# Zeng-Yan/centermask2

Measured on AMD Instinct MI355X. Metric: images/sec whole-node (V2-39-eSE 3x800x1280), higher is better.
Workload: dtype f32; 1 GPU; Full CenterMask2 V-39-eSE (VoVNetV2-FPN + FCOS + CenterROIHeads/SAG-Mask/MaskIoU + ROIAlignV2), bs=8 per GPU, 3x800x1280, end-to-end (BASELINE configs[3]); global_batch=8, per_gpu_batch=8, parallelism=dp1, launch=hip-graph, collective=none, weights=seeded random-init, reference state-dict keys

## Files before the change

centermask2_amd/csrc/detect.hip:

```cpp
#include "cmk_common.hpp"

namespace cmk {

constexpr int SEL_CHUNK = 4096;
constexpr int MAX_LEVELS = 8;

struct SelLevels {
    const float* logits[MAX_LEVELS];
    const float* regctr[MAX_LEVELS];
    int W[MAX_LEVELS];
    int stride[MAX_LEVELS];
    int elems[MAX_LEVELS];
    int blk_begin[MAX_LEVELS + 1];
    int num_levels;
};

__device__ inline float sigmoidf_(float x) { return 1.0f / (1.0f + expf(-x)); }

__device__ inline int find_level(const SelLevels& L, int b) {
    int l = 0;
#pragma unroll
    for (int i = 1; i < MAX_LEVELS; ++i)
        if (i < L.num_levels && b >= L.blk_begin[i]) l = i;
    return l;
}

__device__ inline bool is_candidate(const float* lg, const float* rc, int e, int ne, int C, float thr, int with_ctr, float& p) {
    if (e >= ne) { p = 0.f; return false; }
    p = sigmoidf_(lg[e]);
    if (!with_ctr) return p > thr;
    return p * sigmoidf_(rc[(long)(e / C) * 5 + 4]) > thr;
}

__global__ __launch_bounds__(256) void sel_count_kernel(const SelLevels L, int C, float thr, int with_ctr, int32_t* __restrict__ block_counts) {
    const int b = blockIdx.x, n = blockIdx.y;
    const int l = find_level(L, b);
    const int e0 = (b - L.blk_begin[l]) * SEL_CHUNK;
    const int ne = L.elems[l];
    const float* lg = L.logits[l] + (long)n * ne;
    const float* rc = L.regctr[l] + (long)n * (ne / C) * 5;
    const int lane = threadIdx.x & 63, wave = threadIdx.x >> 6;
    int cnt = 0;
#pragma unroll 4
    for (int it = 0; it < 16; ++it) {
        int e = e0 + wave * 1024 + it * 64 + lane;
        float p;
        bool c = is_candidate(lg, rc, e, ne, C, thr, with_ctr, p);
        cnt += __popcll(__ballot(c));
    }
    __shared__ int wc[4];
    if (lane == 0) wc[wave] = cnt;
    __syncthreads();
    if (threadIdx.x == 0) block_counts[(long)n * gridDim.x + b] = wc[0] + wc[1] + wc[2] + wc[3];
}

__global__ __launch_bounds__(256) void sel_scan_kernel(int32_t* __restrict__ block_counts, int blocks_per_image, int32_t* __restrict__ counts) {
    __shared__ int part[256];
    const int n = blockIdx.x;
    int32_t* bc = block_counts + (long)n * blocks_per_image;
    const int per = cdiv(blocks_per_image, 256);
    const int b0 = threadIdx.x * per, b1 = min(blocks_per_image, b0 + per);
    int s = 0;
    for (int b = b0; b < b1; ++b) s += bc[b];
    part[threadIdx.x] = s;
    __syncthreads();
    if (threadIdx.x == 0) {
        int run = 0;
        for (int i = 0; i < 256; ++i) { int v = part[i]; part[i] = run; run += v; }
        counts[n] = run;
    }
    __syncthreads();
    int run = part[threadIdx.x];
    for (int b = b0; b < b1; ++b) { int v = bc[b]; bc[b] = run; run += v; }
}

__global__ __launch_bounds__(256) void sel_write_kernel(const SelLevels L, int C, float thr, int with_ctr, const int32_t* __restrict__ block_offsets,
                                                       float* __restrict__ cand_box, float* __restrict__ cand_score,
                                                       int32_t* __restrict__ cand_cls, float* __restrict__ cand_loc, int cap) {
    const int b = blockIdx.x, n = blockIdx.y;
    const int l = find_level(L, b);
    const int e0 = (b - L.blk_begin[l]) * SEL_CHUNK;
    const int ne = L.elems[l];
    const float* lg = L.logits[l] + (long)n * ne;
    const float* rc = L.regctr[l] + (long)n * (ne / C) * 5;
    const int Wl = L.W[l];
    const float fstride = (float)L.stride[l];
    const float half = (float)(L.stride[l] / 2);
    const int lane = threadIdx.x & 63, wave = threadIdx.x >> 6;
    const unsigned long long lt = (lane == 0) ? 0ull : (~0ull >> (64 - lane));

    int cnt = 0;
    for (int it = 0; it < 16; ++it) {
        int e = e0 + wave * 1024 + it * 64 + lane;
        float p;
        bool c = is_candidate(lg, rc, e, ne, C, thr, with_ctr, p);
        cnt += __popcll(__ballot(c));
    }
    __shared__ int wc[4];
    if (lane == 0) wc[wave] = cnt;
    __syncthreads();
    int base = block_offsets[(long)n * gridDim.x + b];
    for (int w = 0; w < wave; ++w) base += wc[w];

    for (int it = 0; it < 16; ++it) {
        int e = e0 + wave * 1024 + it * 64 + lane;
        float p;
        const bool c = is_candidate(lg, rc, e, ne, C, thr, with_ctr, p);
        unsigned long long m = __ballot(c);
        int dst = base + __popcll(m & lt);
        base += __popcll(m);
        if (c && dst < cap) {
            int loc = e / C, cls = e - loc * C;
            const float* r = rc + (long)loc * 5;
            float ctr = sigmoidf_(r[4]);
            float score = sqrtf(p * ctr);
            float lx = (float)((loc % Wl) * L.stride[l]) + half;
            float ly = (float)((loc / Wl) * L.stride[l]) + half;
            float r0 = r[0] * fstride, r1 = r[1] * fstride, r2 = r[2] * fstride, r3 = r[3] * fstride;
            long o = (long)n * cap + dst;
            cand_box[o * 4 + 0] = lx - r0;
            cand_box[o * 4 + 1] = ly - r1;
            cand_box[o * 4 + 2] = lx + r2;
            cand_box[o * 4 + 3] = ly + r3;
            cand_score[o] = score;
            cand_cls[o] = cls;
            cand_loc[o * 2 + 0] = lx;
            cand_loc[o * 2 + 1] = ly;
        }
    }
}

constexpr int NT = 1024;
constexpr int NW = NT / 64;
constexpr int MAXK = 1024;

__device__ inline float iou_f(float ax1, float ay1, float ax2, float ay2, float aarea, float bx1, float by1, float bx2, float by2,
                              float barea) {
    float xx1 = fmaxf(ax1, bx1), yy1 = fmaxf(ay1, by1);
    float xx2 = fminf(ax2, bx2), yy2 = fminf(ay2, by2);
    float w = fmaxf(0.0f, xx2 - xx1), h = fmaxf(0.0f, yy2 - yy1);
    float inter = w * h;
    return inter / (aarea + barea - inter);
}

__global__ __launch_bounds__(NT) void nms_topk_kernel(const float* __restrict__ cand_box, const float* __restrict__ cand_score,
                                                     const int32_t* __restrict__ cand_cls, const float* __restrict__ cand_loc,
                                                     const int32_t* __restrict__ counts, int cap, float thr, int topk,
                                                     float* __restrict__ out_box, float* __restrict__ out_score,
                                                     int64_t* __restrict__ out_cls, float* __restrict__ out_loc,
                                                     int32_t* __restrict__ out_idx, int32_t* __restrict__ out_count,
                                                     uint32_t* __restrict__ sort_ws) {
    __shared__ int hist[256];
    __shared__ int base[256];
    __shared__ int wcnt[NW][256];
    __shared__ float red[NW];
    __shared__ float s_maxc;
    __shared__ float kx1[MAXK], ky1[MAXK], kx2[MAXK], ky2[MAXK], karea[MAXK];
    __shared__ int kcls[MAXK];
    __shared__ int s_nkept;

    const int n = blockIdx.x;
    const int tid = threadIdx.x, lane = tid & 63, wave = tid >> 6;
    const int cnt = min(counts[n], cap);
    const float* box = cand_box + (long)n * cap * 4;
    const float* score = cand_score + (long)n * cap;
    const int32_t* cls = cand_cls + (long)n * cap;
    uint32_t* k0 = sort_ws + ((long)n * 4 + 0) * cap;
    uint32_t* v0 = sort_ws + ((long)n * 4 + 1) * cap;
    uint32_t* k1 = sort_ws + ((long)n * 4 + 2) * cap;
    uint32_t* v1 = sort_ws + ((long)n * 4 + 3) * cap;

    float lmax = -INFINITY;
    for (int i = tid; i < cnt; i += NT) {
        k0[i] = ~__float_as_uint(score[i]);
        v0[i] = (uint32_t)i;
        const float* b = box + (long)i * 4;
        lmax = fmaxf(lmax, fmaxf(fmaxf(b[0], b[1]), fmaxf(b[2], b[3])));
    }
    lmax = wave_max(lmax);
    if (lane == 0) red[wave] = lmax;
    __syncthreads();
    if (tid == 0) {
        float m = red[0];
        for (int w = 1; w < NW; ++w) m = fmaxf(m, red[w]);
        s_maxc = m;
        s_nkept = 0;
    }
    __syncthreads();

    const unsigned long long lt = (lane == 0) ? 0ull : (~0ull >> (64 - lane));
    const int NEED = max(2048, 16 * topk);
    int sorted_cnt = cnt;
    for (int attempt = (cnt > 2 * NEED ? 0 : 1); attempt < 2; ++attempt) {
    uint32_t *kin = k0, *vin = v0, *kout = k1, *vout = v1;
    sorted_cnt = cnt;
    if (attempt == 1 && cnt > 2 * NEED) {
        for (int i = tid; i < cnt; i += NT) { k0[i] = ~__float_as_uint(score[i]); v0[i] = (uint32_t)i; }
        __threadfence_block();
        __syncthreads();
    }
    if (attempt == 0) {
        int* hist12 = &wcnt[0][0];
        for (int j = tid; j < 4096; j += NT) hist12[j] = 0;
        __syncthreads();
        for (int i = tid; i < cnt; i += NT) atomicAdd(&hist12[k0[i] >> 20], 1);
        __syncthreads();
        const int h0 = hist12[4 * tid], h1 = hist12[4 * tid + 1], h2 = hist12[4 * tid + 2], h3 = hist12[4 * tid + 3];
        const int mine = h0 + h1 + h2 + h3;
        int incl = mine;
#pragma unroll
        for (int o = 1; o < 64; o <<= 1) { int v = __shfl_up(incl, o, 64); if (lane >= o) incl += v; }
        if (lane == 63) base[wave] = incl;
        __syncthreads();
        int pre = incl - mine;
        for (int w = 0; w < wave; ++w) pre += base[w];
        if (pre < NEED && pre + mine >= NEED) {
            int c = pre + h0, d = 4 * tid;
            if (c < NEED) { c += h1; ++d; }
            if (c < NEED) { c += h2; ++d; }
            if (c < NEED) { c += h3; ++d; }
            hist[0] = d;
            hist[1] = c;
        }
        __syncthreads();
        const uint32_t dmax = (uint32_t)hist[0];
        sorted_cnt = hist[1];
        __syncthreads();
        int run = 0;
        for (int t0 = 0; t0 < cnt; t0 += NT) {
            const int i = t0 + tid;
            const bool take = i < cnt && (k0[i] >> 20) <= dmax;
            const unsigned long long bm = __ballot(take);
            if (lane == 0) base[wave] = __popcll(bm);
            __syncthreads();
            int pos = run + __popcll(bm & lt);
            for (int w = 0; w < wave; ++w) pos += base[w];
            if (take) { k1[pos] = k0[i]; v1[pos] = (uint32_t)i; }
            int tot = 0;
            for (int w = 0; w < NW; ++w) tot += base[w];
            run += tot;
            __syncthreads();
        }
        __threadfence_block();
        __syncthreads();
        kin = k1; vin = v1; kout = k0; vout = v0;
    }
    const int scnt = sorted_cnt;
    for (int pass = 0; pass < 4; ++pass) {
        const int shift = pass * 8;
        if (tid < 256) hist[tid] = 0;
        __syncthreads();
        for (int i = tid; i < scnt; i += NT) atomicAdd(&hist[(kin[i] >> shift) & 255], 1);
        __syncthreads();
        if (tid == 0) {
            int run = 0;
            for (int d = 0; d < 256; ++d) { base[d] = run; run += hist[d]; }
        }
        __syncthreads();
        const bool trivial = false;
        (void)trivial;
        for (int t0 = 0; t0 < scnt; t0 += NT) {
            for (int j = tid; j < NW * 256; j += NT) (&wcnt[0][0])[j] = 0;
            __syncthreads();
            const int i = t0 + tid;
            const bool valid = i < scnt;
            uint32_t key = valid ? kin[i] : 0u, val = valid ? vin[i] : 0u;
            int digit = valid ? (int)((key >> shift) & 255) : 256;
            unsigned long long peers = __ballot(valid);
#pragma unroll
            for (int bit = 0; bit < 8; ++bit) {
                unsigned long long bm = __ballot((digit >> bit) & 1);
                peers &= ((digit >> bit) & 1) ? bm : ~bm;
            }
            int rank = __popcll(peers & lt);
            if (valid && rank == 0) wcnt[wave][digit] = __popcll(peers);
            __syncthreads();
            if (valid) {
                int pre = base[digit];
                for (int w = 0; w < wave; ++w) pre += wcnt[w][digit];
                kout[pre + rank] = key;
                vout[pre + rank] = val;
            }
            __syncthreads();
            if (tid < 256) {
                int s = 0;
                for (int w = 0; w < NW; ++w) s += wcnt[w][tid];
                base[tid] += s;
            }
            __syncthreads();
        }
        uint32_t* t;
        t = kin; kin = kout; kout = t;
        t = vin; vin = vout; vout = t;
        __threadfence_block();
        __syncthreads();
    }
    const uint32_t* order = vin;

    if (wave == 0) {
        const bool per_class = cnt >= 40000;
        const float off_unit = per_class ? 0.0f : (s_maxc + 1.0f);
        int nkept = 0;
        for (int c0 = 0; c0 < scnt && nkept < topk; c0 += 64) {
            const int pos = c0 + lane;
            bool alive = pos < scnt;
            int idx = alive ? (int)order[pos] : 0;
            float x1 = 0, y1 = 0, x2 = 0, y2 = 0, area = 0;
            int mycls = -1;
            if (alive) {
                const float* b = box + (long)idx * 4;
                mycls = cls[idx];
                float off = (float)mycls * off_unit;
                x1 = b[0] + off; y1 = b[1] + off; x2 = b[2] + off; y2 = b[3] + off;
                area = (x2 - x1) * (y2 - y1);
                for (int k = 0; k < nkept; ++k) {
                    if (per_class && kcls[k] != mycls) continue;
                    if (iou_f(kx1[k], ky1[k], kx2[k], ky2[k], karea[k], x1, y1, x2, y2, area) > thr) { alive = false; break; }
                }
            }
            for (int t = 0; t < 64 && nkept < topk; ++t) {
                unsigned long long am = __ballot(alive);
                if (!((am >> t) & 1ull)) continue;
                float tx1 = __shfl(x1, t, 64), ty1 = __shfl(y1, t, 64), tx2 = __shfl(x2, t, 64), ty2 = __shfl(y2, t, 64);
                float tarea = __shfl(area, t, 64);
                int tcls = __shfl(mycls, t, 64);
                int tidx = __shfl(idx, t, 64);
                if (lane == 0) {
                    kx1[nkept] = tx1; ky1[nkept] = ty1; kx2[nkept] = tx2; ky2[nkept] = ty2; karea[nkept] = tarea; kcls[nkept] = tcls;
                    long o = (long)n * topk + nkept;
                    const float* b = box + (long)tidx * 4;
                    out_box[o * 4 + 0] = b[0]; out_box[o * 4 + 1] = b[1]; out_box[o * 4 + 2] = b[2]; out_box[o * 4 + 3] = b[3];
                    out_score[o] = score[tidx];
                    out_cls[o] = (int64_t)tcls;
                    out_loc[o * 2 + 0] = cand_loc[((long)n * cap + tidx) * 2 + 0];
                    out_loc[o * 2 + 1] = cand_loc[((long)n * cap + tidx) * 2 + 1];
                    out_idx[o] = tidx;
                }
                ++nkept;
                if (lane > t && alive && (!per_class || tcls == mycls) &&
                    iou_f(tx1, ty1, tx2, ty2, tarea, x1, y1, x2, y2, area) > thr)
                    alive = false;
                if (lane == t) alive = false;
            }
        }
        if (lane == 0) {
            out_count[n] = nkept;
            s_nkept = nkept;
        }
    }
    __syncthreads();
    if (s_nkept >= topk || sorted_cnt >= cnt) break;
    __syncthreads();
    }
    __syncthreads();
    for (int k = s_nkept + tid; k < topk; k += NT) {
        long o = (long)n * topk + k;
        out_box[o * 4 + 0] = out_box[o * 4 + 1] = out_box[o * 4 + 2] = out_box[o * 4 + 3] = 0.f;
        out_score[o] = 0.f;
        out_cls[o] = 0;
        out_loc[o * 2] = out_loc[o * 2 + 1] = 0.f;
        out_idx[o] = -1;
    }
}

static int fill_levels(const cmk_fcos_level* levels, int num_levels, int C, SelLevels& L) {
    if (num_levels < 1 || num_levels > MAX_LEVELS) return -1;
    int blk = 0;
    L.num_levels = num_levels;
    for (int l = 0; l < MAX_LEVELS; ++l) {
        if (l < num_levels) {
            long e = (long)levels[l].H * levels[l].W * C;
            if (e <= 0 || e > 0x7fffffffL) return -1;
            L.logits[l] = levels[l].logits; L.regctr[l] = levels[l].regctr;
            L.W[l] = levels[l].W; L.stride[l] = levels[l].stride; L.elems[l] = (int)e;
            L.blk_begin[l] = blk;
            blk += (int)((e + SEL_CHUNK - 1) / SEL_CHUNK);
        } else {
            L.logits[l] = nullptr; L.regctr[l] = nullptr; L.W[l] = 1; L.stride[l] = 1; L.elems[l] = 0; L.blk_begin[l] = blk;
        }
    }
    L.blk_begin[MAX_LEVELS] = blk;
    return blk;
}

}

using namespace cmk;

extern "C" int64_t cmk_fcos_select_ws_len(const cmk_fcos_level* levels, int num_levels, int N, int C) {
    SelLevels L;
    int blk = fill_levels(levels, num_levels, C, L);
    return blk < 0 ? -1 : (int64_t)blk * N;
}

extern "C" int cmk_fcos_select(const cmk_fcos_level* levels, int num_levels, int N, int C, float pre_nms_thresh, int thresh_with_ctr, float* cand_box,
                               float* cand_score, int32_t* cand_cls, float* cand_loc, int32_t* counts, int32_t* block_counts,
                               int64_t block_counts_len, int cap, void* stream) {
    if (!levels || !cand_box || !cand_score || !cand_cls || !cand_loc || !counts || !block_counts)
        return fail(CMK_EINVAL, "fcos_select: null pointer%s", "");
    if (N < 1 || C < 1 || cap < 1) return fail(CMK_EINVAL, "fcos_select: bad sizes%s", "");
    SelLevels L;
    int blk = fill_levels(levels, num_levels, C, L);
    if (blk < 0) return fail(CMK_EINVAL, "fcos_select: bad level table%s", "");
    for (int l = 0; l < num_levels; ++l)
        if (!levels[l].logits || !levels[l].regctr) return fail(CMK_EINVAL, "fcos_select: null level pointer%s", "");
    if (block_counts_len < (int64_t)blk * N) return fail(CMK_EINVAL, "fcos_select: workspace too small%s", "");
    hipStream_t st = (hipStream_t)stream;
    hipLaunchKernelGGL(sel_count_kernel, dim3(blk, N), dim3(256), 0, st, L, C, pre_nms_thresh, thresh_with_ctr, block_counts);
    int rc = check_launch("sel_count");
    if (rc) return rc;
    hipLaunchKernelGGL(sel_scan_kernel, dim3(N), dim3(256), 0, st, block_counts, blk, counts);
    rc = check_launch("sel_scan");
    if (rc) return rc;
    hipLaunchKernelGGL(sel_write_kernel, dim3(blk, N), dim3(256), 0, st, L, C, pre_nms_thresh, thresh_with_ctr, block_counts, cand_box, cand_score,
                       cand_cls, cand_loc, cap);
    return check_launch("sel_write");
}

extern "C" int cmk_nms_topk(const float* cand_box, const float* cand_score, const int32_t* cand_cls, const float* cand_loc,
                            const int32_t* counts, int N, int cap, float iou_thr, int topk, float* out_box, float* out_score,
                            int64_t* out_cls, float* out_loc, int32_t* out_idx, int32_t* out_count, uint32_t* sort_ws, void* stream) {
    if (!cand_box || !cand_score || !cand_cls || !cand_loc || !counts || !out_box || !out_score || !out_cls || !out_loc || !out_idx ||
        !out_count || !sort_ws)
        return fail(CMK_EINVAL, "nms_topk: null pointer%s", "");
    if (N < 1 || cap < 1 || topk < 1 || topk > MAXK) return fail(CMK_EINVAL, "nms_topk: need 1 <= topk <= %s%ld", "", (long)MAXK);
    hipLaunchKernelGGL(nms_topk_kernel, dim3(N), dim3(NT), 0, (hipStream_t)stream, cand_box, cand_score, cand_cls, cand_loc, counts, cap,
                       iou_thr, topk, out_box, out_score, out_cls, out_loc, out_idx, out_count, sort_ws);
    return check_launch("nms_topk");
}
```

centermask2_amd/csrc/elementwise.hip:

```cpp
#include "cmk_common.hpp"

namespace cmk {

typedef float f32x4 __attribute__((ext_vector_type(4)));
typedef float f32x16 __attribute__((ext_vector_type(16)));

template <int NB>
__global__ __launch_bounds__(256) void stem_conv_kernel(const float* __restrict__ x, const float* __restrict__ w,
                                                       const float* __restrict__ scale, const float* __restrict__ shift,
                                                       float* __restrict__ y, int N, int H, int W, int Ho, int Wo, long tiles) {
    const int lane = threadIdx.x & 63, wave = threadIdx.x >> 6;
    const int li = lane & 31, hh = lane >> 5;
    constexpr int Cout = NB * 32;
    float b[14][NB], sc[NB], sh[NB];
    int dlt[14], khs[14], kws[14];
#pragma unroll
    for (int s = 0; s < 14; ++s) {
        const int k = 2 * s + hh;
        const int ci = k % 3, t = k / 3, kw = t % 3, kh = t / 3;
        khs[s] = kh - 1; kws[s] = kw - 1;
        dlt[s] = (ci * H + kh - 1) * W + kw - 1;
#pragma unroll
        for (int nb = 0; nb < NB; ++nb) b[s][nb] = k < 27 ? w[k * Cout + nb * 32 + li] : 0.f;
    }
#pragma unroll
    for (int nb = 0; nb < NB; ++nb) { sc[nb] = scale[nb * 32 + li]; sh[nb] = shift[nb * 32 + li]; }
    const long total = (long)N * Ho * Wo;
    const long hw = (long)Ho * Wo;
    for (long tile = (long)blockIdx.x * 4 + wave; tile < tiles; tile += (long)gridDim.x * 4) {
        const long pix = tile * 32 + li;
        const bool pv = pix < total;
        const int n = (int)(pix / hw);
        const int rem = (int)(pix - (long)n * hw);
        const int oh = rem / Wo, ow = rem - oh * Wo;
        const int ih0 = oh * 2, iw0 = ow * 2;
        const float* xb = x + ((long)n * 3 * H + ih0) * W + iw0;
        float av[14];
#pragma unroll
        for (int s = 0; s < 14; ++s) {
            const int ih = ih0 + khs[s], iw = iw0 + kws[s];
            const bool ok = pv && (2 * s + hh < 27) && ih >= 0 && ih < H && iw >= 0 && iw < W;
            av[s] = ok ? xb[dlt[s]] : 0.f;
        }
        f32x16 acc[NB];
#pragma unroll
        for (int nb = 0; nb < NB; ++nb)
#pragma unroll
            for (int r = 0; r < 16; ++r) acc[nb][r] = 0.f;
#pragma unroll
        for (int s = 0; s < 14; ++s)
#pragma unroll
            for (int nb = 0; nb < NB; ++nb) acc[nb] = __builtin_amdgcn_mfma_f32_32x32x2f32(av[s], b[s][nb], acc[nb], 0, 0, 0);
#pragma unroll
        for (int r = 0; r < 16; ++r) {
            const long op = tile * 32 + (r & 3) + 8 * (r >> 2) + 4 * hh;
            if (op < total) {
#pragma unroll
                for (int nb = 0; nb < NB; ++nb) y[op * Cout + nb * 32 + li] = fmaxf(acc[nb][r] * sc[nb] + sh[nb], 0.f);
            }
        }
    }
}

__global__ __launch_bounds__(256) void maxpool3_kernel(const float* __restrict__ x, int x_cs, int x_co, float* __restrict__ y,
                                                      int y_cs, int y_co, int N, int H, int W, int Ho, int Wo, int C4,
                                                      const float* __restrict__ gate) {
    long total = (long)N * Ho * Wo * C4;
    for (long i = (long)blockIdx.x * 256 + threadIdx.x; i < total; i += (long)gridDim.x * 256) {
        int c4 = (int)(i % C4);
        long p = i / C4;
        int ow = (int)(p % Wo);
        int oh = (int)((p / Wo) % Ho);
        int n = (int)(p / ((long)Wo * Ho));
        f32x4 m = {-INFINITY, -INFINITY, -INFINITY, -INFINITY};
#pragma unroll
        for (int kh = 0; kh < 3; ++kh)
#pragma unroll
            for (int kw = 0; kw < 3; ++kw) {
                int ih = oh * 2 + kh, iw = ow * 2 + kw;
                if (ih < H && iw < W) {
                    f32x4 v = *reinterpret_cast<const f32x4*>(x + (((long)n * H + ih) * W + iw) * x_cs + x_co + c4 * 4);
                    m.x = fmaxf(m.x, v.x); m.y = fmaxf(m.y, v.y); m.z = fmaxf(m.z, v.z); m.w = fmaxf(m.w, v.w);
                }
            }
        if (gate) {
            f32x4 g = *reinterpret_cast<const f32x4*>(gate + ((long)n * C4 + c4) * 4);
            m.x *= g.x; m.y *= g.y; m.z *= g.z; m.w *= g.w;
        }
        *reinterpret_cast<f32x4*>(y + p * y_cs + y_co + c4 * 4) = m;
    }
}

__global__ __launch_bounds__(256) void subsample2_kernel(const float* __restrict__ x, int x_cs, int x_co, float* __restrict__ y, int y_cs, int y_co,
                                                        int N, int H, int W, int Ho, int Wo, int C4) {
    long total = (long)N * Ho * Wo * C4;
    for (long i = (long)blockIdx.x * 256 + threadIdx.x; i < total; i += (long)gridDim.x * 256) {
        int c4 = (int)(i % C4);
        long p = i / C4;
        int ow = (int)(p % Wo);
        int oh = (int)((p / Wo) % Ho);
        int n = (int)(p / ((long)Wo * Ho));
        *reinterpret_cast<f32x4*>(y + p * y_cs + y_co + c4 * 4) =
            *reinterpret_cast<const f32x4*>(x + (((long)n * H + 2 * oh) * W + 2 * ow) * x_cs + x_co + c4 * 4);
    }
}

__global__ __launch_bounds__(256) void ese_partial_kernel(const float* __restrict__ x, int x_cs, int x_co, float* __restrict__ ws,
                                                         int HW, int C, int chunks) {
    extern __shared__ float red[];
    const int n = blockIdx.y, chunk = blockIdx.x;
    const int G = C >> 2;
    const int ppl = G >= 256 ? 1 : 256 / G;
    const int per = cdiv(HW, chunks);
    const int p0 = chunk * per, p1 = min(HW, p0 + per);
    const float* xn = x + (long)n * HW * x_cs + x_co;
    for (int gi = threadIdx.x; gi < G * ppl; gi += 256) {
        int g = gi % G, pl = gi / G;
        f32x4 s = {0.f, 0.f, 0.f, 0.f};
        for (int p = p0 + pl; p < p1; p += ppl) {
            f32x4 v = *reinterpret_cast<const f32x4*>(xn + (long)p * x_cs + g * 4);
            s.x += v.x; s.y += v.y; s.z += v.z; s.w += v.w;
        }
        *reinterpret_cast<f32x4*>(red + pl * C + g * 4) = s;
    }
    __syncthreads();
    for (int c = threadIdx.x; c < C; c += 256) {
        float s = 0.f;
        for (int pl = 0; pl < ppl; ++pl) s += red[pl * C + c];
        ws[((long)n * chunks + chunk) * C + c] = s;
    }
}

__global__ __launch_bounds__(256) void ese_fc_kernel(const float* __restrict__ ws, const float* __restrict__ fc_w,
                                                    const float* __restrict__ fc_b, float* __restrict__ gate, int HW, int C,
                                                    int chunks) {
    extern __shared__ double smd[];
    const int n = blockIdx.y;
    const int G = C >> 2;
    const int parts = G >= 256 ? 1 : 256 / G;
    const float* wsn = ws + (long)n * chunks * C;
    for (int gi = threadIdx.x; gi < G * parts; gi += 256) {
        const int g = gi % G, part = gi / G;
        double s0 = 0.0, s1 = 0.0, s2 = 0.0, s3 = 0.0;
#pragma unroll 8
        for (int k = part; k < chunks; k += parts) {
            const f32x4 v = *reinterpret_cast<const f32x4*>(wsn + (long)k * C + g * 4);
            s0 += (double)v.x; s1 += (double)v.y; s2 += (double)v.z; s3 += (double)v.w;
        }
        double* o = smd + part * C + g * 4;
        o[0] = s0; o[1] = s1; o[2] = s2; o[3] = s3;
    }
    __syncthreads();
    for (int c = threadIdx.x; c < C; c += 256) {
        double s = 0.0;
        for (int part = 0; part < parts; ++part) s += smd[part * C + c];
        smd[c] = s / (double)HW;
    }
    __syncthreads();
    const int lane = threadIdx.x & 63, wave = threadIdx.x >> 6;
    for (int o = blockIdx.x * 16 + wave; o < min(C, (int)(blockIdx.x + 1) * 16); o += 4) {
        const float* wr = fc_w + (long)o * C;
        double s = 0.0;
        for (int c = lane * 4; c < C; c += 256) {
            f32x4 wv = *reinterpret_cast<const f32x4*>(wr + c);
            s += (double)wv.x * smd[c] + (double)wv.y * smd[c + 1] + (double)wv.z * smd[c + 2] + (double)wv.w * smd[c + 3];
        }
        s = wave_sum(s);
        if (lane == 0) {
            float v = (float)(s + (double)fc_b[o] + 3.0);
            gate[(long)n * C + o] = fminf(fmaxf(v, 0.f), 6.f) / 6.0f;
        }
    }
}

__global__ __launch_bounds__(256) void ese_fc_pooled_kernel(const float* __restrict__ rec, int rows, const float* __restrict__ fc_w,
                                                           const float* __restrict__ fc_b, float* __restrict__ gate, int HW, int C) {
    extern __shared__ double smd[];
    const int n = blockIdx.y;
    const int G = C >> 2;
    const int parts = G >= 256 ? 1 : 256 / G;
    const long p0 = (long)n * HW;
    const long g0 = p0 / rows, g1 = (p0 + HW - 1) / rows;
    const long first = (g0 * rows == p0) ? 2 * g0 : 2 * g0 + 1;
    for (int gi = threadIdx.x; gi < G * parts; gi += 256) {
        const int g = gi % G, part = gi / G;
        double s0 = 0.0, s1 = 0.0, s2 = 0.0, s3 = 0.0;
        if (part == 0) {
            const f32x4 v = *reinterpret_cast<const f32x4*>(rec + first * C + g * 4);
            s0 = v.x; s1 = v.y; s2 = v.z; s3 = v.w;
        }
#pragma unroll 8
        for (long k = g0 + 1 + part; k <= g1; k += parts) {
            const f32x4 v = *reinterpret_cast<const f32x4*>(rec + 2 * k * C + g * 4);
            s0 += (double)v.x; s1 += (double)v.y; s2 += (double)v.z; s3 += (double)v.w;
        }
        double* o = smd + part * C + g * 4;
        o[0] = s0; o[1] = s1; o[2] = s2; o[3] = s3;
    }
    __syncthreads();
    for (int c = threadIdx.x; c < C; c += 256) {
        double s = 0.0;
        for (int part = 0; part < parts; ++part) s += smd[part * C + c];
        smd[c] = s / (double)HW;
    }
    __syncthreads();
    const int lane = threadIdx.x & 63, wave = threadIdx.x >> 6;
    for (int o = blockIdx.x * 16 + wave; o < min(C, (int)(blockIdx.x + 1) * 16); o += 4) {
        const float* wr = fc_w + (long)o * C;
        double s = 0.0;
        for (int c = lane * 4; c < C; c += 256) {
            f32x4 wv = *reinterpret_cast<const f32x4*>(wr + c);
            s += (double)wv.x * smd[c] + (double)wv.y * smd[c + 1] + (double)wv.z * smd[c + 2] + (double)wv.w * smd[c + 3];
        }
        s = wave_sum(s);
        if (lane == 0) {
            float v = (float)(s + (double)fc_b[o] + 3.0);
            gate[(long)n * C + o] = fminf(fmaxf(v, 0.f), 6.f) / 6.0f;
        }
    }
}

__global__ __launch_bounds__(256) void ese_scale_kernel(const float* __restrict__ x, int x_cs, int x_co, const float* __restrict__ gate,
                                                       const float* __restrict__ idn, int id_cs, int id_co, float* __restrict__ y,
                                                       int y_cs, int y_co, int N, int HW, int C4) {
    long total = (long)N * HW * C4;
    for (long i = (long)blockIdx.x * 256 + threadIdx.x; i < total; i += (long)gridDim.x * 256) {
        int c4 = (int)(i % C4);
        long p = i / C4;
        int n = (int)(p / HW);
        f32x4 v = *reinterpret_cast<const f32x4*>(x + p * x_cs + x_co + c4 * 4);
        f32x4 g = *reinterpret_cast<const f32x4*>(gate + (long)n * C4 * 4 + c4 * 4);
        f32x4 o = {v.x * g.x, v.y * g.y, v.z * g.z, v.w * g.w};
        if (idn) {
            f32x4 d = *reinterpret_cast<const f32x4*>(idn + p * id_cs + id_co + c4 * 4);
            o.x += d.x; o.y += d.y; o.z += d.z; o.w += d.w;
        }
        *reinterpret_cast<f32x4*>(y + p * y_cs + y_co + c4 * 4) = o;
    }
}

}

using namespace cmk;

extern "C" int cmk_stem_conv_nchw3(const float* x, const float* w, const float* scale, const float* shift, float* y, int N, int H,
                                   int W, int Cout, void* stream) {
    if (!x || !w || !scale || !shift || !y) return fail(CMK_EINVAL, "stem: null pointer%s", "");
    if (Cout != 32 && Cout != 64 && Cout != 128) return fail(CMK_EINVAL, "stem: Cout (%s%ld) must be 32, 64 or 128", "", (long)Cout);
    int Ho = (H - 1) / 2 + 1, Wo = (W - 1) / 2 + 1;
    long total = (long)N * Ho * Wo;
    if ((long)3 * H * W >= (1L << 31)) return fail(CMK_EINVAL, "stem: image too large%s", "");
    long tiles = (total + 31) / 32;
    unsigned grid = (unsigned)std::min<long>((tiles + 3) / 4, 256 * 16);
    if (Cout == 32)
        hipLaunchKernelGGL(stem_conv_kernel<1>, dim3(grid), dim3(256), 0, (hipStream_t)stream, x, w, scale, shift, y, N, H, W, Ho, Wo, tiles);
    else if (Cout == 64)
        hipLaunchKernelGGL(stem_conv_kernel<2>, dim3(grid), dim3(256), 0, (hipStream_t)stream, x, w, scale, shift, y, N, H, W, Ho, Wo, tiles);
    else
        hipLaunchKernelGGL(stem_conv_kernel<4>, dim3(grid), dim3(256), 0, (hipStream_t)stream, x, w, scale, shift, y, N, H, W, Ho, Wo, tiles);
    return check_launch("stem_conv");
}

extern "C" int cmk_maxpool3x3s2_ceil_nhwc(const float* x, int x_cs, int x_co, float* y, int y_cs, int y_co, int N, int H, int W, int C,
                                          const float* gate, void* stream) {
    if (!x || !y) return fail(CMK_EINVAL, "maxpool: null pointer%s", "");
    if ((C & 3) || (x_cs & 3) || (x_co & 3) || (y_cs & 3) || (y_co & 3)) return fail(CMK_EINVAL, "maxpool: channels must be multiples of 4%s", "");
    if (H < 3 || W < 3) return fail(CMK_EINVAL, "maxpool: input smaller than the window%s", "");
    int Ho = (H - 3 + 1) / 2 + 1, Wo = (W - 3 + 1) / 2 + 1;
    if ((Ho - 1) * 2 >= H) --Ho;
    if ((Wo - 1) * 2 >= W) --Wo;
    long total = (long)N * Ho * Wo * (C >> 2);
    hipLaunchKernelGGL(maxpool3_kernel, dim3(stream_grid(total)), dim3(256), 0, (hipStream_t)stream, x, x_cs, x_co, y, y_cs, y_co, N, H, W,
                       Ho, Wo, C >> 2, gate);
    return check_launch("maxpool3");
}

extern "C" int cmk_maxpool1x1s2_nhwc(const float* x, int x_cs, int x_co, float* y, int y_cs, int y_co, int N, int H, int W, int C, void* stream) {
    if (!x || !y) return fail(CMK_EINVAL, "maxpool1x1s2: null pointer%s", "");
    if ((C & 3) || (x_cs & 3) || (x_co & 3) || (y_cs & 3) || (y_co & 3) || N < 1 || H < 1 || W < 1)
        return fail(CMK_EINVAL, "maxpool1x1s2: channels must be multiples of 4, N, H, W >= 1%s", "");
    const int Ho = (H - 1) / 2 + 1, Wo = (W - 1) / 2 + 1;
    long total = (long)N * Ho * Wo * (C >> 2);
    hipLaunchKernelGGL(subsample2_kernel, dim3(stream_grid(total)), dim3(256), 0, (hipStream_t)stream, x, x_cs, x_co, y, y_cs, y_co, N, H, W, Ho, Wo,
                       C >> 2);
    return check_launch("maxpool1x1s2");
}

extern "C" int cmk_ese_gate(const float* x, int x_cs, int x_co, const float* fc_w, const float* fc_b, float* gate, float* ws,
                            int ws_chunks, int N, int HW, int C, void* stream) {
    if (!x || !fc_w || !fc_b || !gate || !ws) return fail(CMK_EINVAL, "ese_gate: null pointer%s", "");
    if ((C & 3) || (x_cs & 3) || (x_co & 3) || ws_chunks < 1) return fail(CMK_EINVAL, "ese_gate: bad shape%s", "");
    int G = C >> 2;
    int ppl = G >= 256 ? 1 : 256 / G;
    size_t lds1 = (size_t)ppl * C * sizeof(float);
    hipLaunchKernelGGL(ese_partial_kernel, dim3(ws_chunks, N), dim3(256), lds1, (hipStream_t)stream, x, x_cs, x_co, ws, HW, C, ws_chunks);
    int rc = check_launch("ese_partial");
    if (rc) return rc;
    hipLaunchKernelGGL(ese_fc_kernel, dim3(cdiv(C, 16), N), dim3(256), 2 * lds1 , (hipStream_t)stream, ws, fc_w, fc_b,
                       gate, HW, C, ws_chunks);
    return check_launch("ese_fc");
}

extern "C" int cmk_ese_gate_pooled(const float* pool_ws, int rows, const float* fc_w, const float* fc_b, float* gate, int N, int HW, int C, void* stream) {
    if (!pool_ws || !fc_w || !fc_b || !gate) return fail(CMK_EINVAL, "ese_gate_pooled: null pointer%s", "");
    if ((C & 3) || rows < 1 || HW < rows || N < 1) return fail(CMK_EINVAL, "ese_gate_pooled: bad shape (C %% 4, H*W >= rows)%s", "");
    const int G = C >> 2;
    const int parts = G >= 256 ? 1 : 256 / G;
    hipLaunchKernelGGL(ese_fc_pooled_kernel, dim3(cdiv(C, 16), N), dim3(256), (size_t)parts * C * sizeof(double), (hipStream_t)stream, pool_ws, rows,
                       fc_w, fc_b, gate, HW, C);
    return check_launch("ese_fc_pooled");
}

extern "C" int cmk_ese_scale(const float* x, int x_cs, int x_co, const float* gate, const float* identity, int id_cs, int id_co, float* y,
                             int y_cs, int y_co, int N, int HW, int C, void* stream) {
    if (!x || !gate || !y) return fail(CMK_EINVAL, "ese_scale: null pointer%s", "");
    if ((C & 3) || (x_cs & 3) || (x_co & 3) || (y_cs & 3) || (y_co & 3) || (id_cs & 3) || (id_co & 3))
        return fail(CMK_EINVAL, "ese_scale: channels must be multiples of 4%s", "");
    long total = (long)N * HW * (C >> 2);
    hipLaunchKernelGGL(ese_scale_kernel, dim3(stream_grid(total)), dim3(256), 0, (hipStream_t)stream, x, x_cs, x_co, gate, identity, id_cs,
                       id_co, y, y_cs, y_co, N, HW, C >> 2);
    return check_launch("ese_scale");
}

__global__ __launch_bounds__(256) void upsample2x_add_kernel(float* __restrict__ y, const float* __restrict__ c, int N, int H, int W, int Hc, int Wc, int C4) {
    long total = (long)N * H * W * C4;
    for (long i = (long)blockIdx.x * 256 + threadIdx.x; i < total; i += (long)gridDim.x * 256) {
        int c4 = (int)(i % C4);
        long p = i / C4;
        int w = (int)(p % W);
        int h = (int)((p / W) % H);
        int n = (int)(p / ((long)W * H));
        const f32x4 a = *reinterpret_cast<const f32x4*>(y + i * 4);
        const f32x4 b = *reinterpret_cast<const f32x4*>(c + ((((long)n * Hc + (h >> 1)) * Wc + (w >> 1)) * C4 + c4) * 4);
        *reinterpret_cast<f32x4*>(y + i * 4) = f32x4{a.x + b.x, a.y + b.y, a.z + b.z, a.w + b.w};
    }
}

extern "C" int cmk_upsample2x_add_nhwc(float* y, const float* coarse, int N, int H, int W, int Hc, int Wc, int C, void* stream) {
    if (!y || !coarse) return fail(CMK_EINVAL, "upsample2x_add: null pointer%s", "");
    if ((C & 3) || N < 1 || H < 1 || W < 1 || Hc * 2 < H || Wc * 2 < W) return fail(CMK_EINVAL, "upsample2x_add: C %% 4 == 0 and a coarse map of at least half the size%s", "");
    long total = (long)N * H * W * (C >> 2);
    hipLaunchKernelGGL(upsample2x_add_kernel, dim3(stream_grid(total)), dim3(256), 0, (hipStream_t)stream, y, coarse, N, H, W, Hc, Wc, C >> 2);
    return check_launch("upsample2x_add");
}
```

Baseline: 374.1 images/sec.

## Fuse radix histograms into the load pass and cut barriers in NMS and eSE FC

The NMS top-k kernel now builds all four 8-bit radix histograms in the same pass that loads keys or compacts them, and scans them once instead of re-counting per pass. The prefix compaction uses a two-pass per-wave count and write with no per-chunk barriers, and reads scores directly rather than staging keys first. Kept-box output writes are deferred to a parallel loop after NMS, and the wave-serial candidate loop now jumps to set bits with ffs. Separately, the eSE FC gate computation processes four outputs per wave with unrolled weight loads, and the pooled reduction batches 16 loads per iteration to expose more memory parallelism. These kernels are a small part of the end-to-end detector, so their effect on whole-model throughput is limited.

```diff
diff --git a/centermask2_amd/csrc/detect.hip b/centermask2_amd/csrc/detect.hip
--- a/centermask2_amd/csrc/detect.hip
+++ b/centermask2_amd/csrc/detect.hip
@@ -150,13 +150,14 @@
                                                      int64_t* __restrict__ out_cls, float* __restrict__ out_loc,
                                                      int32_t* __restrict__ out_idx, int32_t* __restrict__ out_count,
                                                      uint32_t* __restrict__ sort_ws) {
-    __shared__ int hist[256];
-    __shared__ int base[256];
+    __shared__ int hist4[4][256];
+    __shared__ int sel[2];
+    __shared__ int wtot[NW];
     __shared__ int wcnt[NW][256];
     __shared__ float red[NW];
     __shared__ float s_maxc;
     __shared__ float kx1[MAXK], ky1[MAXK], kx2[MAXK], ky2[MAXK], karea[MAXK];
-    __shared__ int kcls[MAXK];
+    __shared__ int kcls[MAXK], kidx[MAXK];
     __shared__ int s_nkept;
 
     const int n = blockIdx.x;
@@ -169,16 +170,31 @@
     uint32_t* v0 = sort_ws + ((long)n * 4 + 1) * cap;
     uint32_t* k1 = sort_ws + ((long)n * 4 + 2) * cap;
     uint32_t* v1 = sort_ws + ((long)n * 4 + 3) * cap;
-
+    int* hist12 = &wcnt[0][0];
+
+    const int NEED = max(2048, 16 * topk);
+    const bool try_prefix = cnt > 2 * NEED;
+
+    for (int j = tid; j < NW * 256; j += NT) hist12[j] = 0;
+    (&hist4[0][0])[tid] = 0;
+    __syncthreads();
     float lmax = -INFINITY;
     for (int i = tid; i < cnt; i += NT) {
-        k0[i] = ~__float_as_uint(score[i]);
-        v0[i] = (uint32_t)i;
+        const uint32_t key = ~__float_as_uint(score[i]);
+        if (try_prefix) {
+            atomicAdd(&hist12[key >> 20], 1);
+        } else {
+            k0[i] = key;
+            v0[i] = (uint32_t)i;
+            atomicAdd(&hist4[0][key & 255], 1); atomicAdd(&hist4[1][(key >> 8) & 255], 1);
+            atomicAdd(&hist4[2][(key >> 16) & 255], 1); atomicAdd(&hist4[3][key >> 24], 1);
+        }
         const float* b = box + (long)i * 4;
         lmax = fmaxf(lmax, fmaxf(fmaxf(b[0], b[1]), fmaxf(b[2], b[3])));
     }
     lmax = wave_max(lmax);
     if (lane == 0) red[wave] = lmax;
+    __threadfence_block();
     __syncthreads();
     if (tid == 0) {
         float m = red[0];
@@ -189,79 +205,91 @@
     __syncthreads();
 
     const unsigned long long lt = (lane == 0) ? 0ull : (~0ull >> (64 - lane));
-    const int NEED = max(2048, 16 * topk);
     int sorted_cnt = cnt;
-    for (int attempt = (cnt > 2 * NEED ? 0 : 1); attempt < 2; ++attempt) {
+    for (int attempt = (try_prefix ? 0 : 1); attempt < 2; ++attempt) {
     uint32_t *kin = k0, *vin = v0, *kout = k1, *vout = v1;
     sorted_cnt = cnt;
-    if (attempt == 1 && cnt > 2 * NEED) {
-        for (int i = tid; i < cnt; i += NT) { k0[i] = ~__float_as_uint(score[i]); v0[i] = (uint32_t)i; }
+    if (attempt == 1 && try_prefix) {
+        (&hist4[0][0])[tid] = 0;
+        __syncthreads();
+        for (int i = tid; i < cnt; i += NT) {
+            const uint32_t key = ~__float_as_uint(score[i]);
+            k0[i] = key;
+            v0[i] = (uint32_t)i;
+            atomicAdd(&hist4[0][key & 255], 1); atomicAdd(&hist4[1][(key >> 8) & 255], 1);
+            atomicAdd(&hist4[2][(key >> 16) & 255], 1); atomicAdd(&hist4[3][key >> 24], 1);
+        }
         __threadfence_block();
         __syncthreads();
     }
     if (attempt == 0) {
-        int* hist12 = &wcnt[0][0];
-        for (int j = tid; j < 4096; j += NT) hist12[j] = 0;
-        __syncthreads();
-        for (int i = tid; i < cnt; i += NT) atomicAdd(&hist12[k0[i] >> 20], 1);
-        __syncthreads();
         const int h0 = hist12[4 * tid], h1 = hist12[4 * tid + 1], h2 = hist12[4 * tid + 2], h3 = hist12[4 * tid + 3];
         const int mine = h0 + h1 + h2 + h3;
         int incl = mine;
 #pragma unroll
         for (int o = 1; o < 64; o <<= 1) { int v = __shfl_up(incl, o, 64); if (lane >= o) incl += v; }
-        if (lane == 63) base[wave] = incl;
+        if (lane == 63) wtot[wave] = incl;
         __syncthreads();
         int pre = incl - mine;
-        for (int w = 0; w < wave; ++w) pre += base[w];
+        for (int w = 0; w < wave; ++w) pre += wtot[w];
         if (pre < NEED && pre + mine >= NEED) {
             int c = pre + h0, d = 4 * tid;
             if (c < NEED) { c += h1; ++d; }
             if (c < NEED) { c += h2; ++d; }
             if (c < NEED) { c += h3; ++d; }
-            hist[0] = d;
-            hist[1] = c;
-        }
-        __syncthreads();
-        const uint32_t dmax = (uint32_t)hist[0];
-        sorted_cnt = hist[1];
-        __syncthreads();
-        int run = 0;
-        for (int t0 = 0; t0 < cnt; t0 += NT) {
-            const int i = t0 + tid;
-            const bool take = i < cnt && (k0[i] >> 20) <= dmax;
+            sel[0] = d;
+            sel[1] = c;
+        }
+        hist12[4 * tid] = 0; hist12[4 * tid + 1] = 0; hist12[4 * tid + 2] = 0; hist12[4 * tid + 3] = 0;
+        __syncthreads();
+        const uint32_t dmax = (uint32_t)sel[0];
+        sorted_cnt = sel[1];
+        const int per = ((cnt + NW * 64 - 1) / (NW * 64)) * 64;
+        const int wb = min(cnt, wave * per), we = min(cnt, wb + per);
+        int mycount = 0;
+        for (int i0 = wb; i0 < we; i0 += 64) {
+            const int i = i0 + lane;
+            const bool take = i < we && ((~__float_as_uint(score[min(i, we - 1)])) >> 20) <= dmax;
+            mycount += __popcll(__ballot(take));
+        }
+        if (lane == 0) wtot[wave] = mycount;
+        __syncthreads();
+        int pos = 0;
+        for (int w = 0; w < wave; ++w) pos += wtot[w];
+        for (int i0 = wb; i0 < we; i0 += 64) {
+            const int i = i0 + lane;
+            const uint32_t key = ~__float_as_uint(score[min(i, we - 1)]);
+            const bool take = i < we && (key >> 20) <= dmax;
             const unsigned long long bm = __ballot(take);
-            if (lane == 0) base[wave] = __popcll(bm);
-            __syncthreads();
-            int pos = run + __popcll(bm & lt);
-            for (int w = 0; w < wave; ++w) pos += base[w];
-            if (take) { k1[pos] = k0[i]; v1[pos] = (uint32_t)i; }
-            int tot = 0;
-            for (int w = 0; w < NW; ++w) tot += base[w];
-            run += tot;
-            __syncthreads();
+            if (take) {
+                const int p = pos + __popcll(bm & lt);
+                k1[p] = key;
+                v1[p] = (uint32_t)i;
+                atomicAdd(&hist4[0][key & 255], 1); atomicAdd(&hist4[1][(key >> 8) & 255], 1);
+                atomicAdd(&hist4[2][(key >> 16) & 255], 1); atomicAdd(&hist4[3][key >> 24], 1);
+            }
+            pos += __popcll(bm);
         }
         __threadfence_block();
         __syncthreads();
         kin = k1; vin = v1; kout = k0; vout = v0;
     }
     const int scnt = sorted_cnt;
+    if (wave < 4) {
+        int* h = hist4[wave];
+        const int a0 = h[4 * lane], a1 = h[4 * lane + 1], a2 = h[4 * lane + 2], a3 = h[4 * lane + 3];
+        const int mine = a0 + a1 + a2 + a3;
+        int incl = mine;
+#pragma unroll
+        for (int o = 1; o < 64; o <<= 1) { int v = __shfl_up(incl, o, 64); if (lane >= o) incl += v; }
+        const int pre = incl - mine;
+        h[4 * lane] = pre; h[4 * lane + 1] = pre + a0; h[4 * lane + 2] = pre + a0 + a1; h[4 * lane + 3] = pre + a0 + a1 + a2;
+    }
+    __syncthreads();
     for (int pass = 0; pass < 4; ++pass) {
         const int shift = pass * 8;
-        if (tid < 256) hist[tid] = 0;
-        __syncthreads();
-        for (int i = tid; i < scnt; i += NT) atomicAdd(&hist[(kin[i] >> shift) & 255], 1);
-        __syncthreads();
-        if (tid == 0) {
-            int run = 0;
-            for (int d = 0; d < 256; ++d) { base[d] = run; run += hist[d]; }
-        }
-        __syncthreads();
-        const bool trivial = false;
-        (void)trivial;
+        int* base = hist4[pass];
         for (int t0 = 0; t0 < scnt; t0 += NT) {
-            for (int j = tid; j < NW * 256; j += NT) (&wcnt[0][0])[j] = 0;
-            __syncthreads();
             const int i = t0 + tid;
             const bool valid = i < scnt;
             uint32_t key = valid ? kin[i] : 0u, val = valid ? vin[i] : 0u;
@@ -284,7 +312,7 @@
             __syncthreads();
             if (tid < 256) {
                 int s = 0;
-                for (int w = 0; w < NW; ++w) s += wcnt[w][tid];
+                for (int w = 0; w < NW; ++w) { s += wcnt[w][tid]; wcnt[w][tid] = 0; }
                 base[tid] += s;
             }
             __syncthreads();
@@ -318,23 +346,15 @@
                     if (iou_f(kx1[k], ky1[k], kx2[k], ky2[k], karea[k], x1, y1, x2, y2, area) > thr) { alive = false; break; }
                 }
             }
-            for (int t = 0; t < 64 && nkept < topk; ++t) {
-                unsigned long long am = __ballot(alive);
-                if (!((am >> t) & 1ull)) continue;
+            for (unsigned long long am = __ballot(alive); am != 0ull && nkept < topk; am = __ballot(alive)) {
+                const int t = __ffsll((long long)am) - 1;
                 float tx1 = __shfl(x1, t, 64), ty1 = __shfl(y1, t, 64), tx2 = __shfl(x2, t, 64), ty2 = __shfl(y2, t, 64);
                 float tarea = __shfl(area, t, 64);
                 int tcls = __shfl(mycls, t, 64);
                 int tidx = __shfl(idx, t, 64);
                 if (lane == 0) {
                     kx1[nkept] = tx1; ky1[nkept] = ty1; kx2[nkept] = tx2; ky2[nkept] = ty2; karea[nkept] = tarea; kcls[nkept] = tcls;
-                    long o = (long)n * topk + nkept;
-                    const float* b = box + (long)tidx * 4;
-                    out_box[o * 4 + 0] = b[0]; out_box[o * 4 + 1] = b[1]; out_box[o * 4 + 2] = b[2]; out_box[o * 4 + 3] = b[3];
-                    out_score[o] = score[tidx];
-                    out_cls[o] = (int64_t)tcls;
-                    out_loc[o * 2 + 0] = cand_loc[((long)n * cap + tidx) * 2 + 0];
-                    out_loc[o * 2 + 1] = cand_loc[((long)n * cap + tidx) * 2 + 1];
-                    out_idx[o] = tidx;
+                    kidx[nkept] = tidx;
                 }
                 ++nkept;
                 if (lane > t && alive && (!per_class || tcls == mycls) &&
@@ -353,6 +373,17 @@
     __syncthreads();
     }
     __syncthreads();
+    for (int k = tid; k < s_nkept; k += NT) {
+        const long o = (long)n * topk + k;
+        const int tidx = kidx[k];
+        const float* b = box + (long)tidx * 4;
+        out_box[o * 4 + 0] = b[0]; out_box[o * 4 + 1] = b[1]; out_box[o * 4 + 2] = b[2]; out_box[o * 4 + 3] = b[3];
+        out_score[o] = score[tidx];
+        out_cls[o] = (int64_t)kcls[k];
+        out_loc[o * 2 + 0] = cand_loc[((long)n * cap + tidx) * 2 + 0];
+        out_loc[o * 2 + 1] = cand_loc[((long)n * cap + tidx) * 2 + 1];
+        out_idx[o] = tidx;
+    }
     for (int k = s_nkept + tid; k < topk; k += NT) {
         long o = (long)n * topk + k;
         out_box[o * 4 + 0] = out_box[o * 4 + 1] = out_box[o * 4 + 2] = out_box[o * 4 + 3] = 0.f;
diff --git a/centermask2_amd/csrc/elementwise.hip b/centermask2_amd/csrc/elementwise.hip
--- a/centermask2_amd/csrc/elementwise.hip
+++ b/centermask2_amd/csrc/elementwise.hip
@@ -131,6 +131,41 @@
     }
 }
 
+__device__ inline void ese_fc_outputs(const double* smd, const float* __restrict__ fc_w, const float* __restrict__ fc_b,
+                                      float* __restrict__ gate_n, int C) {
+    constexpr int NO = 4, KU = 4;
+    const int lane = threadIdx.x & 63, wave = threadIdx.x >> 6;
+    const int ob = blockIdx.x * 16 + wave;
+    double s[NO] = {0.0, 0.0, 0.0, 0.0};
+    for (int c0 = lane * 4; c0 < C; c0 += 256 * KU) {
+        f32x4 wv[NO][KU];
+#pragma unroll
+        for (int j = 0; j < NO; ++j)
+#pragma unroll
+            for (int k = 0; k < KU; ++k)
+                wv[j][k] = *reinterpret_cast<const f32x4*>(fc_w + (long)min(ob + 4 * j, C - 1) * C + min(c0 + 256 * k, C - 4));
+#pragma unroll
+        for (int k = 0; k < KU; ++k) {
+            const int c = c0 + 256 * k;
+            if (c < C) {
+#pragma unroll
+                for (int j = 0; j < NO; ++j)
+                    s[j] += (double)wv[j][k].x * smd[c] + (double)wv[j][k].y * smd[c + 1] + (double)wv[j][k].z * smd[c + 2] +
+                            (double)wv[j][k].w * smd[c + 3];
+            }
+        }
+    }
+#pragma unroll
+    for (int j = 0; j < NO; ++j) {
+        const int o = ob + 4 * j;
+        const double t = wave_sum(s[j]);
+        if (lane == 0 && o < min(C, (int)(blockIdx.x + 1) * 16)) {
+            float v = (float)(t + (double)fc_b[o] + 3.0);
+            gate_n[o] = fminf(fmaxf(v, 0.f), 6.f) / 6.0f;
+        }
+    }
+}
+
 __global__ __launch_bounds__(256) void ese_fc_kernel(const float* __restrict__ ws, const float* __restrict__ fc_w,
                                                     const float* __restrict__ fc_b, float* __restrict__ gate, int HW, int C,
                                                     int chunks) {
@@ -157,20 +192,7 @@
         smd[c] = s / (double)HW;
     }
     __syncthreads();
-    const int lane = threadIdx.x & 63, wave = threadIdx.x >> 6;
-    for (int o = blockIdx.x * 16 + wave; o < min(C, (int)(blockIdx.x + 1) * 16); o += 4) {
-        const float* wr = fc_w + (long)o * C;
-        double s = 0.0;
-        for (int c = lane * 4; c < C; c += 256) {
-            f32x4 wv = *reinterpret_cast<const f32x4*>(wr + c);
-            s += (double)wv.x * smd[c] + (double)wv.y * smd[c + 1] + (double)wv.z * smd[c + 2] + (double)wv.w * smd[c + 3];
-        }
-        s = wave_sum(s);
-        if (lane == 0) {
-            float v = (float)(s + (double)fc_b[o] + 3.0);
-            gate[(long)n * C + o] = fminf(fmaxf(v, 0.f), 6.f) / 6.0f;
-        }
-    }
+    ese_fc_outputs(smd, fc_w, fc_b, gate + (long)n * C, C);
 }
 
 __global__ __launch_bounds__(256) void ese_fc_pooled_kernel(const float* __restrict__ rec, int rows, const float* __restrict__ fc_w,
@@ -189,10 +211,13 @@
             const f32x4 v = *reinterpret_cast<const f32x4*>(rec + first * C + g * 4);
             s0 = v.x; s1 = v.y; s2 = v.z; s3 = v.w;
         }
-#pragma unroll 8
-        for (long k = g0 + 1 + part; k <= g1; k += parts) {
-            const f32x4 v = *reinterpret_cast<const f32x4*>(rec + 2 * k * C + g * 4);
-            s0 += (double)v.x; s1 += (double)v.y; s2 += (double)v.z; s3 += (double)v.w;
+        for (long k = g0 + 1 + part; k <= g1; k += 16 * parts) {
+            f32x4 v[16];
+#pragma unroll
+            for (int j = 0; j < 16; ++j) v[j] = *reinterpret_cast<const f32x4*>(rec + 2 * min(k + (long)j * parts, g1) * C + g * 4);
+#pragma unroll
+            for (int j = 0; j < 16; ++j)
+                if (k + (long)j * parts <= g1) { s0 += (double)v[j].x; s1 += (double)v[j].y; s2 += (double)v[j].z; s3 += (double)v[j].w; }
         }
         double* o = smd + part * C + g * 4;
         o[0] = s0; o[1] = s1; o[2] = s2; o[3] = s3;
@@ -204,20 +229,7 @@
         smd[c] = s / (double)HW;
     }
     __syncthreads();
-    const int lane = threadIdx.x & 63, wave = threadIdx.x >> 6;
-    for (int o = blockIdx.x * 16 + wave; o < min(C, (int)(blockIdx.x + 1) * 16); o += 4) {
-        const float* wr = fc_w + (long)o * C;
-        double s = 0.0;
-        for (int c = lane * 4; c < C; c += 256) {
-            f32x4 wv = *reinterpret_cast<const f32x4*>(wr + c);
-            s += (double)wv.x * smd[c] + (double)wv.y * smd[c + 1] + (double)wv.z * smd[c + 2] + (double)wv.w * smd[c + 3];
-        }
-        s = wave_sum(s);
-        if (lane == 0) {
-            float v = (float)(s + (double)fc_b[o] + 3.0);
-            gate[(long)n * C + o] = fminf(fmaxf(v, 0.f), 6.f) / 6.0f;
-        }
-    }
+    ese_fc_outputs(smd, fc_w, fc_b, gate + (long)n * C, C);
 }
 
 __global__ __launch_bounds__(256) void ese_scale_kernel(const float* __restrict__ x, int x_cs, int x_co, const float* __restrict__ gate,
```

Result: no change. 377.1 images/sec, median of 6 (+0.8%).
